# JiehongLin/SAM-6D

Measured on NVIDIA H100. Metric: poses/sec, higher is better.
Workload: dtype bf16

## Files before the change

include/sam6d_b200.h:

```cpp
#ifndef SAM6D_B200_H
#define SAM6D_B200_H

#ifdef __cplusplus
extern "C" {
#endif


int sam6d_fps(const float* xyz, int b, int n, int m, float* temp, int* idx, void* stream);
int sam6d_fps_single_cta(const float* xyz, int b, int n, int m, float* temp, int* idx, void* stream);

int sam6d_gather_points(const float* points, const int* idx, int b, int c, int n, int m, float* out, void* stream);

int sam6d_gather_rows(const float* src, const int* idx, int b, int n, int m, int c, long long src_bstride, float* out,
                      void* stream);
int sam6d_gather_rows_bf16_f32(const void* src, const int* idx, int b, int n, int m, int c, long long src_bstride, float* out,
                               void* stream);

int sam6d_ball_query(const float* new_xyz, const float* xyz, int b, int n, int m, float radius, int nsample, int* idx,
                     int* cnt, void* stream);
int sam6d_ball_query_pair(const float* new_xyz, const float* xyz, int b, int n, int m, float radius_a, int nsample_a,
                          float radius_b, int nsample_b, int* idx_a, int* idx_b, int* cnt_a, int* cnt_b, void* stream);

int sam6d_group_points(const float* points, const int* idx, int b, int c, int n, int np, int ns, float* out, void* stream);

// ... 125 lines not shown
                     float* lse, void* out, int out_is_bf16, long long out_ld, void* stream);
int sam6d_attn_merge_key(const void* Q, long long q_ld, int q_col0, const void* K, long long k_ld, int k_col0, int k_brows,
                         int key_row, const void* Vt, long long vt_ld, int key_col, const float* lse, int B, int H, int Sq,
                         float scale, void* out, long long out_ld, void* stream);
int sam6d_transpose_tokens_bf16(const void* src, long long ld, int col0, int C, int nB, int L, int N1, void* out, void* stream);
int sam6d_linattn_kv(const float* Kf, long long k_ld, long long k_bs, const float* V, long long v_ld, long long v_bs, int B,
                     int H, int J, float* KV, float* KS, void* stream);
int sam6d_linattn_apply(const float* Qf, long long q_rpb, long long q_bs, long long q_ld, const float* KV, const float* KS,
                        int B, int H, float* X, long long x_bs, long long x_ld, void* stream);
int sam6d_linattn_kv_pack(const float* Kf, long long k_ld, long long k_bs, const float* V, long long v_ld, long long v_bs, int B,
                          int J, void* blob, float* KS, void* stream);
int sam6d_linattn_tc(const void* Q, long long q_ld, long long q_bs, const void* blob, const float* KS,
                     const float* softplus_scale, int B, int rpb, void* X, long long x_ld, long long x_bs, void* stream);

int sam6d_coarse_assign(const float* A, int B, int S, float* W, float* w1, void* stream);
int sam6d_coarse_sample(const float* W, int B, int L, const float* rand, int nr, int* idx, void* stream);
int sam6d_coarse_hypotheses(const int* idx, const float* pts1, const float* pts2, int B, int n, int n1, float* Rt,
                            float* resid, void* stream);
int sam6d_topk_smallest(const float* v, int B, int n, int k, int* out, void* stream);
int sam6d_coarse_select(const float* Rt, const int* top, int B, int n1, int n2, const float* pts1, const float* w1, int n,
                        const float* model, int nm, float* scores, float* R, float* t, void* stream);


int sam6d_pe_mlp_max(const float* pts, const int* idx, const int* cnt, int B, int N, int ns, const float* W1,
                     const float* B1, const float* W2, const float* B2, const float* W3, const float* B3, float* out,
                     int out_ld, int out_off, void* stream);
int sam6d_pe_mlp_max_tc(const float* pts, const int* idx, int B, int N, int ns, const float* W1, const float* B1,
                        const void* W2_bf16, const float* B2, const void* W3_bf16, const float* B3, void* out, int out_is_bf16,
                        int out_ld, int out_off, void* stream);
int sam6d_fine_assign(const float* A, int B, int S, int ld, float shift, const float* pts2, float* rsum, float* csum, float* cpart,
                      int* cpi, int* lab1, int* lab2, float* wts, float* pred, void* stream);
int sam6d_fine_pass_tc(const void* Fa, const void* Fb, int B, int S, float alpha, float shift, int mode, const float* row_f,
                       const float* col_f, int ld_f, const float* q4, float* out_inv, int* lab, float* wts, float* pred, void* stream);
int sam6d_fine_masked_points(const int* lab2, const float* pts2, int B, int S, int ld, float* q4, void* stream);
int sam6d_weighted_procrustes(const float* src, const float* ref, const float* wts, int B, int N, float weight_thresh,
                              float eps, float* R, float* t, void* stream);
int sam6d_pose_score(const float* pts1, const int* lab1, int B, int N, const float* R, const float* t, const float* model,
                     int nm, float dis_thres, const float* radius, float* score, float* t_scaled, void* stream);

int sam6d_bilinear_gather(const void* up, int up_is_bf16, const long long* choose, int B, int K, int G, int sub, int C, int H, int W,
                          float* out, void* stream);

int sam6d_attn_relpos(const float* qkv, long long tok_ld, int nW, int Hs, int Ws, int nH, int head_dim, const float* rel_h,
                      const float* rel_w, float scale, void* out, int out_is_bf16, long long out_ld, void* stream);

int sam6d_attn_global_tc(const void* qkv, long long ld, const void* Vt, long long vt_ld, const void* rel_blob, int B, int H, int grid,
                         float scale, void* out, int out_is_bf16, long long out_ld, void* stream);
int sam6d_attn_global_tc_ex(const void* qkv, long long ld, const void* Vt, long long vt_ld, const void* rel_blob, int B, int H, int grid,
                            int head_dim, float scale, void* out, int out_is_bf16, long long out_ld, void* stream);

int sam6d_template_score_agg(const float* Qn, const float* Rn, int P, int O, int T, int C, int aggregation, float* sim_out,
                             float* obj_score, int* obj_tmpl, int* best_obj, float* best_score, int* best_tmpl, void* stream);
int sam6d_template_score(const float* Qn, const float* Rn, int P, int O, int T, int C, float* sim_out, float* obj_score,
                         int* best_obj, float* best_score, int* best_tmpl, void* stream);


int sam6d_render_meshes(const float* verts, const int* faces, const int* mesh_info, int O, int n_verts, int n_faces,
                        const unsigned char* vcol, const float* uv, const unsigned char* tex, const long long* tex_off,
                        const float* base_color, const float* poses, int T, float fx, float fy, float cx, float cy, int H, int W,
                        float znear, float ambient, int* vrec, unsigned long long* vis, int* big, int big_cap, int* counters,
                        unsigned char* rgb, unsigned char* mask, void* xyz, int* tri, float* depth, void* stream);


int sam6d_bop_mssd_mspd(const float* est, const float* gt, const int* pair_obj, const float* K, int P, const float* verts,
                        const int* vert_off, const float* syms, const int* sym_off, int O, int max_sym, float* out, void* stream);
int sam6d_bop_vsd_counts(const float* depth_est, const float* depth_gt, const float* depth_test, const int* pair_img, int P,
// ... 23 lines not shown
```

sam6d_b200/_lib.py:

```python
import ctypes
import os
import re

_HERE = os.path.dirname(os.path.abspath(__file__))
HEADER = os.path.join(os.path.dirname(_HERE), "include", "sam6d_b200.h")
LIB_PATH = os.path.join(_HERE, "libsam6d_b200.so")

_CTYPES = {
    "int": ctypes.c_int,
    "long long": ctypes.c_longlong,
    "float": ctypes.c_float,
    "double": ctypes.c_double,
}


def parse_header(path: str = HEADER):
    text = open(path).read()
    text = re.sub(r"/\*.*?\*/", "", text, flags=re.S)
    protos = {}
    for m in re.finditer(r"(const char\*|int)\s+(sam6d_\w+)\s*\(([^)]*)\)\s*;", text):
        ret, name, args = m.group(1), m.group(2), m.group(3)
        argl = []
        for a in [x.strip() for x in args.split(",")]:
            if a in ("void", ""):
# ... 2 lines not shown
                argl.append((ctypes.c_void_p, a.split("*")[-1].strip()))
            else:
                typ, nm = a.rsplit(" ", 1)
                argl.append((_CTYPES[typ.strip()], nm))
        protos[name] = (ctypes.c_char_p if ret != "int" else ctypes.c_int, argl)
    return protos


class Sam6dError(RuntimeError):
    pass


_lib = None
_protos = None


def lib():
    global _lib, _protos
    if _lib is None:
        if not os.path.exists(LIB_PATH):
            raise Sam6dError(
                f"{LIB_PATH} not found: build it with `python -m sam6d_b200.build` "
                "(or __graft_entry__.build()); sam6d_b200 has no CPU or eager fallback")
        _lib = ctypes.CDLL(LIB_PATH)
        _protos = parse_header()
        for name, (ret, args) in _protos.items():
            fn = getattr(_lib, name)
            fn.restype = ret
            fn.argtypes = [t for t, _ in args]
    return _lib


_launches = 0
_MULTI = {"sam6d_fine_assign": 6, "sam6d_coarse_select": 2, "sam6d_geo_embed_tc": 2, "sam6d_render_meshes": 4, "sam6d_yolo_masks": 2,
          "sam6d_mask_rle_count": 2, "sam6d_template_score_agg": 2, "sam6d_template_score": 2,
          "sam6d_pbr_reference_crops": 2}
_timed = {}


def launch_count() -> int:
    return _launches


def add_launches(n: int):
    global _launches
    _launches += int(n)


def time_kernel(name: str, enable: bool = True):
    if enable:
        _timed[name] = []
    else:
        _timed.pop(name, None)


def timed_events(name: str):
    return _timed.get(name, [])


def call(name: str, *args):
    global _launches
    fn = getattr(lib(), name)
    rec = _timed.get(name)
    if rec is not None:
        import torch
        e0, e1 = torch.cuda.Event(enable_timing=True), torch.cuda.Event(enable_timing=True)
        e0.record()
# ... 16 lines not shown
```

sam6d_b200/csrc/coarse.cu:

```cuda
#include "common.cuh"
#include "svd3.cuh"

namespace {

constexpr int ASSIGN_THREADS = 1024;
__global__ void __launch_bounds__(ASSIGN_THREADS) coarse_assign_kernel(const float* __restrict__ A, int S, float* __restrict__ W,
                                                            float* __restrict__ w1out) {
  extern __shared__ float sm[];
  float* a = sm;
  float* rmax = a + S * S;
  float* rsum = rmax + S;
  float* cmax = rsum + S;
  float* csum = cmax + S;
  int* lab1 = (int*)(csum + S);
  int* lab2 = lab1 + S;
  const int b = blockIdx.x, tid = threadIdx.x, lane = tid & 31, warp = tid >> 5;
  const float* Ab = A + (size_t)b * S * S;
  for (int e = tid; e < S * S; e += ASSIGN_THREADS) a[e] = Ab[e];
  __syncthreads();
  for (int i = warp; i < S; i += ASSIGN_THREADS / 32) {
    float m = -INFINITY;
    for (int j = lane; j < S; j += 32) m = fmaxf(m, a[i * S + j]);
    m = warp_max(m);
    float s = 0.f;
// ... 14 lines not shown
    float v = a[e];
    a[e] = (expf(v - rmax[i]) / rsum[i]) * (expf(v - cmax[j]) / csum[j]);
  }
  __syncthreads();
  for (int i = warp; i < S; i += ASSIGN_THREADS / 32) {
    float bv = -INFINITY; int bi = 0x7fffffff;
    for (int j = lane; j < S; j += 32) argmax_first(bv, bi, a[i * S + j], j);
    warp_argmax_first(bv, bi);
    if (lane == 0) lab1[i] = bi;
  }
  for (int j = tid; j < S; j += ASSIGN_THREADS) {
    float bv = -INFINITY; int bi = 0;
    for (int i = 0; i < S; ++i) { float v = a[i * S + j]; if (v > bv) { bv = v; bi = i; } }
    lab2[j] = bi;
  }
  __syncthreads();
  const int n = S - 1;
  float* Wb = W + (size_t)b * n * n;
  for (int e = tid; e < n * n; e += ASSIGN_THREADS) {
    int i = e / n, j = e - i * n;
    float v = a[(i + 1) * S + (j + 1)];
    v = v * (lab1[i + 1] > 0 ? 1.f : 0.f) * (lab2[j + 1] > 0 ? 1.f : 0.f);
    Wb[e] = v * sqrtf(v);
  }
  for (int i = tid; i < n; i += ASSIGN_THREADS) w1out[(size_t)b * n + i] = lab1[i + 1] > 0 ? 1.f : 0.f;
}

__global__ void __launch_bounds__(1024) coarse_sample_kernel(const float* __restrict__ W, int L, const float* __restrict__ rand,
                                                             int nr, int* __restrict__ idx_out) {
  extern __shared__ float cdf[];
  __shared__ double part[1024];
  const int b = blockIdx.x, tid = threadIdx.x;
  const float* Wb = W + (size_t)b * L;
  const int per = (L + 1023) / 1024;
  const int beg = min(tid * per, L), end = min(beg + per, L);
  double s = 0.0;
  for (int i = beg; i < end; ++i) s += (double)Wb[i];
  part[tid] = s;
  __syncthreads();
  for (int o = 1; o < 1024; o <<= 1) {
    double v = (tid >= o) ? part[tid - o] : 0.0;
    __syncthreads();
    part[tid] += v;
    __syncthreads();
  }
  double run = (tid == 0) ? 0.0 : part[tid - 1];
  for (int i = beg; i < end; ++i) { run += (double)Wb[i]; cdf[i] = (float)run; }
  __syncthreads();
  const float denom = cdf[L - 1] + 1e-8f;
  __syncthreads();
  for (int i = tid; i < L; i += 1024) cdf[i] = cdf[i] / denom;
  __syncthreads();
  for (int r = tid; r < nr; r += 1024) {
    float v = rand[(size_t)b * nr + r];
    int lo = 0, hi = L;
    while (lo < hi) {
      int mid = (lo + hi) >> 1;
      if (cdf[mid] < v) lo = mid + 1; else hi = mid;
    }
    idx_out[(size_t)b * nr + r] = lo;
  }
}

__global__ void __launch_bounds__(128) coarse_hyp_kernel(const int* __restrict__ idx, const float* __restrict__ pts1,
                                                         const float* __restrict__ pts2, int n, int n1, float* __restrict__ Rt,
                                                         float* __restrict__ resid) {
  const int b = blockIdx.y;
  const int hpt = blockIdx.x * blockDim.x + threadIdx.x;
  if (hpt >= n1) return;
  const int* id = idx + ((size_t)b * n1 + hpt) * 3;
  float p1[3][3], p2[3][3];
  int i1s[3], i2s[3];
#pragma unroll
  for (int k = 0; k < 3; ++k) {
    int v = id[k];
    int i1 = min(v / n, n - 1), i2 = min(v % n, n - 1);
    i1s[k] = i1; i2s[k] = i2;
    const float* a = pts1 + ((size_t)b * n + i1) * 3;
    const float* c = pts2 + ((size_t)b * n + i2) * 3;
#pragma unroll
// ... 24 lines not shown
  if (rank0) {
#pragma unroll
    for (int i = 0; i < 3; ++i)
#pragma unroll
      for (int j = 0; j < 3; ++j) Rd[i][j] = (i == j) ? 1.0 : 0.0;
  } else {
    procrustes_rotation(H, Rd, rank1);
  }
  float R[3][3], t[3];
#pragma unroll
  for (int i = 0; i < 3; ++i)
#pragma unroll
    for (int j = 0; j < 3; ++j) R[i][j] = (float)Rd[i][j];
#pragma unroll
  for (int i = 0; i < 3; ++i) t[i] = cr[i] - (R[i][0] * cs[0] + R[i][1] * cs[1] + R[i][2] * cs[2]);
  float rs = 0.f;
#pragma unroll
  for (int k = 0; k < 3; ++k) {
    float x = p1[k][0] - t[0], y = p1[k][1] - t[1], z = p1[k][2] - t[2];
    float ex = x * R[0][0] + y * R[1][0] + z * R[2][0] - p2[k][0];
    float ey = x * R[0][1] + y * R[1][1] + z * R[2][1] - p2[k][1];
    float ez = x * R[0][2] + y * R[1][2] + z * R[2][2] - p2[k][2];
    rs += sqrtf(ex * ex + ey * ey + ez * ez);
  }
  float* o = Rt + ((size_t)b * n1 + hpt) * 12;
#pragma unroll
  for (int i = 0; i < 3; ++i)
#pragma unroll
    for (int j = 0; j < 3; ++j) o[i * 3 + j] = R[i][j];
  o[9] = t[0]; o[10] = t[1]; o[11] = t[2];
  resid[(size_t)b * n1 + hpt] = rs / 3.f;
}

__global__ void __launch_bounds__(1024) topk_smallest_kernel(const float* __restrict__ v, int n, int npow2, int k,
                                                             int* __restrict__ out) {
  extern __shared__ unsigned long long keys[];
  const int b = blockIdx.x, tid = threadIdx.x;
  for (int i = tid; i < npow2; i += 1024) {
    unsigned long long key = ~0ull;
    if (i < n) {
      float f = v[(size_t)b * n + i];
      unsigned u = __float_as_uint(f);
      u = (u & 0x80000000u) ? ~u : (u | 0x80000000u);
      key = ((unsigned long long)u << 32) | (unsigned)i;
    }
    keys[i] = key;
  }
  __syncthreads();
  for (int size = 2; size <= npow2; size <<= 1) {
    for (int stride = size >> 1; stride > 0; stride >>= 1) {
      for (int i = tid; i < npow2 / 2; i += 1024) {
        int lo = 2 * i - (i & (stride - 1));
        int hi = lo + stride;
        bool asc = ((lo & size) == 0);
        unsigned long long a = keys[lo], c = keys[hi];
        if ((a > c) == asc) { keys[lo] = c; keys[hi] = a; }
      }
      __syncthreads();
    }
  }
  for (int i = tid; i < k; i += 1024) out[(size_t)b * k + i] = (int)(keys[i] & 0xffffffffu);
}

constexpr int SEL_PP = 4, SEL_THREADS = 224;
__device__ __forceinline__ float min3f(float a, float b, float c) { return fminf(fminf(a, b), c); }
__global__ void __launch_bounds__(SEL_THREADS) coarse_select_kernel(const float* __restrict__ Rt, const int* __restrict__ top, int n1,
                                                                    int n2, const float* __restrict__ pts1, const float* __restrict__ w1,
                                                                    int n, const float* __restrict__ model, int nm,
                                                                    float* __restrict__ scores) {
  extern __shared__ float4 smq[];
  __shared__ float red[2 * SEL_PP][SEL_THREADS / 32];
  __shared__ float rts[SEL_PP][12];
  const int pose0 = blockIdx.x * SEL_PP, b = blockIdx.y, tid = threadIdx.x;
  for (int i = tid; i < nm; i += SEL_THREADS) {
    const float* q = model + ((size_t)b * nm + i) * 3;
    const float x = q[0], y = q[1], z = q[2];
    smq[i] = make_float4(x, y, z, x * x + y * y + z * z);
  }
  if (tid < SEL_PP * 12) {
    const int pp = tid / 12, e = tid - pp * 12;
    const int pose = min(pose0 + pp, n2 - 1);
    rts[pp][e] = Rt[((size_t)b * n1 + top[(size_t)b * n2 + pose]) * 12 + e];
  }
  __syncthreads();
  float num = 0.f, den[SEL_PP];
#pragma unroll
  for (int pp = 0; pp < SEL_PP; ++pp) den[pp] = 0.f;
  for (int i = tid; i < n; i += SEL_THREADS) {
    const float* p = pts1 + ((size_t)b * n + i) * 3;
    const float px = p[0], py = p[1], pz = p[2];
    float ax[SEL_PP], ay[SEL_PP], az[SEL_PP], x2[SEL_PP], best[SEL_PP];
#pragma unroll
    for (int pp = 0; pp < SEL_PP; ++pp) {
      const float* R = rts[pp];
      const float x = px - R[9], y = py - R[10], z = pz - R[11];
      const float tx = x * R[0] + y * R[3] + z * R[6];
      const float ty = x * R[1] + y * R[4] + z * R[7];
// ... 53 lines not shown
S6_API int sam6d_coarse_assign(const float* A, int B, int S, float* W, float* w1, void* stream) {
  S6_REQUIRE(A && W && w1 && B >= 0 && S >= 2);
  if (B == 0) return 0;
  size_t smem = ((size_t)S * S + 6 * S) * sizeof(float);
  S6_REQUIRE(smem <= 220 * 1024);
  S6_CHECK(cudaFuncSetAttribute(coarse_assign_kernel, cudaFuncAttributeMaxDynamicSharedMemorySize, (int)smem));
  coarse_assign_kernel<<<B, ASSIGN_THREADS, smem, s6_stream(stream)>>>(A, S, W, w1);
  S6_LAUNCH_CHECK();
  return 0;
}

S6_API int sam6d_coarse_sample(const float* W, int B, int L, const float* rand, int nr, int* idx, void* stream) {
  S6_REQUIRE(W && rand && idx && B >= 0 && L > 0 && nr >= 0);
  if (B == 0 || nr == 0) return 0;
  size_t smem = (size_t)L * sizeof(float);
  S6_REQUIRE(smem <= 200 * 1024);
  S6_CHECK(cudaFuncSetAttribute(coarse_sample_kernel, cudaFuncAttributeMaxDynamicSharedMemorySize, (int)smem));
  coarse_sample_kernel<<<B, 1024, smem, s6_stream(stream)>>>(W, L, rand, nr, idx);
  S6_LAUNCH_CHECK();
  return 0;
}

S6_API int sam6d_coarse_hypotheses(const int* idx, const float* pts1, const float* pts2, int B, int n, int n1, float* Rt,
                                   float* resid, void* stream) {
  S6_REQUIRE(idx && pts1 && pts2 && Rt && resid && B >= 0 && n > 0 && n1 >= 0);
  if (B == 0 || n1 == 0) return 0;
  dim3 grid(s6_cdiv(n1, 128), B);
  coarse_hyp_kernel<<<grid, 128, 0, s6_stream(stream)>>>(idx, pts1, pts2, n, n1, Rt, resid);
  S6_LAUNCH_CHECK();
  return 0;
}

S6_API int sam6d_topk_smallest(const float* v, int B, int n, int k, int* out, void* stream) {
  S6_REQUIRE(v && out && B >= 0 && n > 0 && k > 0 && k <= n);
  if (B == 0) return 0;
  int npow2 = 2;
  while (npow2 < n) npow2 <<= 1;
  size_t smem = (size_t)npow2 * sizeof(unsigned long long);
  S6_REQUIRE(smem <= 200 * 1024);
  S6_CHECK(cudaFuncSetAttribute(topk_smallest_kernel, cudaFuncAttributeMaxDynamicSharedMemorySize, (int)smem));
  topk_smallest_kernel<<<B, 1024, smem, s6_stream(stream)>>>(v, n, npow2, k, out);
  S6_LAUNCH_CHECK();
  return 0;
}

S6_API int sam6d_coarse_select(const float* Rt, const int* top, int B, int n1, int n2, const float* pts1, const float* w1, int n,
                               const float* model, int nm, float* scores, float* R, float* t, void* stream) {
  S6_REQUIRE(Rt && top && pts1 && w1 && model && scores && R && t && B >= 0 && n > 0 && nm > 0 && n2 > 0);
  if (B == 0) return 0;
  size_t smem = (size_t)nm * 4 * sizeof(float);
  S6_REQUIRE(smem <= 200 * 1024);
  S6_CHECK(cudaFuncSetAttribute(coarse_select_kernel, cudaFuncAttributeMaxDynamicSharedMemorySize, (int)smem));
  dim3 grid(s6_cdiv(n2, SEL_PP), B);
  coarse_select_kernel<<<grid, SEL_THREADS, smem, s6_stream(stream)>>>(Rt, top, n1, n2, pts1, w1, n, model, nm, scores);
  S6_LAUNCH_CHECK();
  coarse_pick_kernel<<<B, 32, 0, s6_stream(stream)>>>(scores, top, Rt, n1, n2, R, t);
  S6_LAUNCH_CHECK();
  return 0;
}
```

sam6d_b200/csrc/fine_tc.cu:

```cuda
#include "common.cuh"
#include "tc.cuh"

namespace {

constexpr int BM = 128, BN = 256, BK = 64, KB = 4, STAGES = 4;
constexpr int A_KB = BM * BK * 2, B_KB = BN * BK * 2;
constexpr int CONSUMERS = 256, NUM_THREADS = CONSUMERS + 128;
constexpr int SMEM_BYTES = KB * A_KB + STAGES * B_KB + 1024;
constexpr float LOG2E = 1.4426950408889634f;

struct FArgs {
  int B, S, mode, ld_f;
  float a2, s2;
  const float* row_f;
  const float* col_f;
  const float4* q4;
  float* out_inv;
  int* lab;
  float* wts; float* pred;
};

__device__ __forceinline__ float ex2(float x) {
  float y;
  asm("ex2.approx.ftz.f32 %0, %1;" : "=f"(y) : "f"(x));
  return y;
}

template <int MODE>
__global__ void __launch_bounds__(NUM_THREADS, 1) fine_pass_kernel(const __grid_constant__ CUtensorMap tmA, const __grid_constant__ CUtensorMap tmB, FArgs g) {
  extern __shared__ __align__(1024) uint8_t smem_raw[];
  uint8_t* smem = reinterpret_cast<uint8_t*>((reinterpret_cast<uintptr_t>(smem_raw) + 1023) & ~(uintptr_t)1023);
  uint8_t* a_res = smem;
  uint8_t* ring = smem + KB * A_KB;
  __shared__ __align__(8) uint64_t a_full, a_empty, full_bar[STAGES], empty_bar[STAGES];
  __shared__ float sc[2][BN];
  __shared__ __align__(16) float4 sq[2][BN];

  const int tid = threadIdx.x, warp = tid >> 5, lane = tid & 31;
  const int m_tiles = (g.S + BM - 1) / BM, n_tiles = (g.S + BN - 1) / BN;
  const int items = g.B * m_tiles;

  if (tid == 0) {
    tc::mbar_init(&a_full, 1); tc::mbar_init(&a_empty, CONSUMERS / 32);
    for (int s = 0; s < STAGES; ++s) { tc::mbar_init(&full_bar[s], 1); tc::mbar_init(&empty_bar[s], CONSUMERS / 32); }
    tc::mbar_fence_init();
    tc::tma_prefetch_desc(&tmA);
    tc::tma_prefetch_desc(&tmB);
  }
  __syncthreads();

  if (warp >= CONSUMERS / 32) {
    tc::producer_regs();
    if (tid == CONSUMERS) {
      long long gk = 0;
      int it = 0;
      for (int item = blockIdx.x; item < items; item += gridDim.x, ++it) {
        const int b = item / m_tiles, mt = item - b * m_tiles;
        tc::mbar_wait(&a_empty, (uint32_t)((it & 1) ^ 1));
        tc::mbar_arrive_expect_tx(&a_full, KB * A_KB);
        for (int kb = 0; kb < KB; ++kb) tc::tma_load_2d(&tmA, &a_full, a_res + kb * A_KB, kb * BK, b * g.S + mt * BM);
        for (int nt = 0; nt < n_tiles; ++nt)
          for (int kb = 0; kb < KB; ++kb, ++gk) {
            const int s = (int)(gk % STAGES);
            tc::mbar_wait(&empty_bar[s], (uint32_t)(((gk / STAGES) & 1) ^ 1));
            tc::mbar_arrive_expect_tx(&full_bar[s], B_KB);
            tc::tma_load_2d(&tmB, &full_bar[s], ring + s * B_KB, kb * BK, b * g.S + nt * BN);
          }
      }
    }
    return;
  }
  tc::consumer_regs();
  const int wg = warp >> 2, w = warp & 3;
  const uint32_t a_addr = tc::smem_u32(a_res) + wg * (64 * 128);
  long long gk = 0, tcount = 0;
  int it = 0;
  for (int item = blockIdx.x; item < items; item += gridDim.x, ++it) {
    const int b = item / m_tiles, mt = item - b * m_tiles;
    float rf[2] = {0.f, 0.f};
#pragma unroll
    for (int hr = 0; hr < 2; ++hr) {
      const int i = mt * BM + wg * 64 + tc::frag_row(2 * hr, w, lane);
      if (MODE != 0 && i < g.S) rf[hr] = g.row_f[(size_t)b * g.ld_f + i];
    }
    const float* cf = (MODE != 0) ? g.col_f + (size_t)b * g.ld_f : nullptr;
    const float4* q4 = (MODE == 2) ? g.q4 + (size_t)b * g.ld_f : nullptr;
    float sum[2] = {0.f, 0.f}, bv[2] = {-INFINITY, -INFINITY}, ws[2] = {0.f, 0.f}, px[2] = {0.f, 0.f}, py[2] = {0.f, 0.f}, pz[2] = {0.f, 0.f};
    int bi[2] = {0x7fffffff, 0x7fffffff};
    tc::mbar_wait(&a_full, (uint32_t)(it & 1));
    for (int nt = 0; nt < n_tiles; ++nt, ++tcount) {
      const int buf = (int)(tcount & 1);
      if (MODE != 0) {
        const int j = nt * BN + tid;
        sc[buf][tid] = (j < g.S) ? cf[j] : 0.f;
        if (MODE == 2) sq[buf][tid] = (j < g.S) ? q4[j] : make_float4(0.f, 0.f, 0.f, 0.f);
        tc::named_bar(1, CONSUMERS);
      }
      float acc[BN / 2];
      int prev = -1;
      for (int kb = 0; kb < KB; ++kb, ++gk) {
        const int s = (int)(gk % STAGES);
        tc::mbar_wait(&full_bar[s], (uint32_t)((gk / STAGES) & 1));
        const uint32_t b_addr = tc::smem_u32(ring + s * B_KB);
        tc::wg_fence();
#pragma unroll
        for (int k = 0; k < BK / 16; ++k)
          tc::wgmma_bf16<BN>(acc, tc::wg_desc(a_addr + kb * A_KB + k * 32), tc::wg_desc(b_addr + k * 32), (kb | k) ? 1u : 0u);
        tc::wg_commit();
        if (prev >= 0) {
          tc::wg_wait<1>();
          if (lane == 0) tc::mbar_arrive(&empty_bar[prev]);
        }
        prev = s;
      }
      tc::wg_wait<0>();
      if (lane == 0) tc::mbar_arrive(&empty_bar[prev]);
      if (nt == n_tiles - 1 && lane == 0) tc::mbar_arrive(&a_empty);
#pragma unroll
      for (int e = 0; e < BN / 2; ++e) {
        const int hr = (e >> 1) & 1, cl = tc::frag_col(e, lane), j = nt * BN + cl;
        const float ev = (j < g.S) ? ex2(fmaf(acc[e], g.a2, -g.s2)) : 0.f;
        if (MODE == 0) {
          sum[hr] += ev;
        } else {
          const float p = (ev * rf[hr]) * (ev * sc[buf][cl]);
          if (p > bv[hr]) { bv[hr] = p; bi[hr] = j; }
          if (MODE == 2) {
            const float4 q = sq[buf][cl];
            const float pm = p * q.w;
            ws[hr] += pm; px[hr] = fmaf(pm, q.x, px[hr]); py[hr] = fmaf(pm, q.y, py[hr]); pz[hr] = fmaf(pm, q.z, pz[hr]);
          }
        }
      }
    }
#pragma unroll
    for (int hr = 0; hr < 2; ++hr) {
      const int i = mt * BM + wg * 64 + tc::frag_row(2 * hr, w, lane);
      if (MODE == 0) {
        const float t = tc::quad_sum(sum[hr]);
        if ((lane & 3) == 0 && i < g.S) g.out_inv[(size_t)b * g.ld_f + i] = 1.f / t;
      } else {
#pragma unroll
        for (int o = 1; o <= 2; o <<= 1) {
          const float ov = __shfl_xor_sync(0xffffffffu, bv[hr], o);
          const int oi = __shfl_xor_sync(0xffffffffu, bi[hr], o);
          if (ov > bv[hr] || (ov == bv[hr] && oi < bi[hr])) { bv[hr] = ov; bi[hr] = oi; }
        }
        float ww = 0.f, qx = 0.f, qy = 0.f, qz = 0.f;
        if (MODE == 2) { ww = tc::quad_sum(ws[hr]); qx = tc::quad_sum(px[hr]); qy = tc::quad_sum(py[hr]); qz = tc::quad_sum(pz[hr]); }
        if ((lane & 3) == 0 && i < g.S) {
          int lb = bi[hr];
          if (lb == 0x7fffffff) lb = 0;
          g.lab[(size_t)b * g.S + i] = lb;
          if (MODE == 2 && i >= 1) {
            if (lb == 0) { ww = 0.f; qx = 0.f; qy = 0.f; qz = 0.f; }
            const size_t o = (size_t)b * (g.S - 1) + (i - 1);
            const float d = ww + 1e-6f;
            g.wts[o] = ww;
            g.pred[o * 3 + 0] = qx / d; g.pred[o * 3 + 1] = qy / d; g.pred[o * 3 + 2] = qz / d;
          }
        }
      }
    }
  }
}

__global__ void fine_masked_points_kernel(const int* __restrict__ lab2, const float* __restrict__ pts2, int S, int ld, float4* __restrict__ q4) {
  const int b = blockIdx.y, j = blockIdx.x * blockDim.x + threadIdx.x;
  if (j >= ld) return;
  float4 q = make_float4(0.f, 0.f, 0.f, 0.f);
  if (j >= 1 && j < S && lab2[(size_t)b * S + j] > 0) {
    const float* p = pts2 + ((size_t)b * (S - 1) + (j - 1)) * 3;
    q = make_float4(p[0], p[1], p[2], 1.f);
  }
  q4[(size_t)b * ld + j] = q;
}

}

S6_API int sam6d_fine_pass_tc(const void* Fa, const void* Fb, int B, int S, float alpha, float shift, int mode, const float* row_f,
                              const float* col_f, int ld_f, const float* q4, float* out_inv, int* lab, float* wts, float* pred,
                              void* stream) {
  S6_REQUIRE(Fa && Fb && B >= 0 && S >= 2 && mode >= 0 && mode <= 2 && ld_f >= S);
  S6_REQUIRE(((reinterpret_cast<uintptr_t>(Fa) | reinterpret_cast<uintptr_t>(Fb)) & 15) == 0 && (long long)B * S < 2000000000LL);
  if (mode == 0) S6_REQUIRE(out_inv != nullptr);
  if (mode >= 1) S6_REQUIRE(row_f && col_f && lab);
  if (mode == 2) S6_REQUIRE(q4 && wts && pred && (reinterpret_cast<uintptr_t>(q4) & 15) == 0);
  if (B == 0) return 0;
  CUtensorMap tmA, tmB;
  int rc = tc::make_map_2d(&tmA, Fa, (long long)B * S, 256, 256, 64, BM);
  if (rc) return rc;
  rc = tc::make_map_2d(&tmB, Fb, (long long)B * S, 256, 256, 64, BN);
  if (rc) return rc;
  int grid;
  S6_CHECK(s6_persistent_grid(B * s6_cdiv(S, BM), 1, &grid));
  FArgs g{B, S, mode, ld_f, alpha * LOG2E, shift * LOG2E, row_f, col_f, reinterpret_cast<const float4*>(q4), out_inv, lab, wts, pred};
  cudaStream_t st = s6_stream(stream);
#define FINE_LAUNCH(M)                                                                                              \
  do {                                                                                                              \
    S6_CHECK(cudaFuncSetAttribute(fine_pass_kernel<M>, cudaFuncAttributeMaxDynamicSharedMemorySize, SMEM_BYTES));   \
    fine_pass_kernel<M><<<grid, NUM_THREADS, SMEM_BYTES, st>>>(tmA, tmB, g);                                        \
  } while (0)
  if (mode == 0) FINE_LAUNCH(0); else if (mode == 1) FINE_LAUNCH(1); else FINE_LAUNCH(2);
#undef FINE_LAUNCH
  S6_LAUNCH_CHECK();
  return 0;
}

S6_API int sam6d_fine_masked_points(const int* lab2, const float* pts2, int B, int S, int ld, float* q4, void* stream) {
  S6_REQUIRE(lab2 && pts2 && q4 && B >= 0 && S >= 2 && ld >= S && (reinterpret_cast<uintptr_t>(q4) & 15) == 0);
  if (B == 0) return 0;
  dim3 grid(s6_cdiv(ld, 256), B);
  fine_masked_points_kernel<<<grid, 256, 0, s6_stream(stream)>>>(lab2, pts2, S, ld, reinterpret_cast<float4*>(q4));
  S6_LAUNCH_CHECK();
  return 0;
}
```

sam6d_b200/ops.py:

```python
import ctypes
from typing import Optional, Tuple

import torch

from . import _lib

Tensor = torch.Tensor


def _check(t: Tensor, dtype, name: str, ndim: Optional[int] = None):
    if not isinstance(t, torch.Tensor):
        raise RuntimeError(f"{name} must be a torch.Tensor")
    if not t.is_cuda:
        raise RuntimeError(f"{name} must be a CUDA tensor (CPU not supported)")
    if t.dtype != dtype:
        raise RuntimeError(f"{name} must be {dtype}, got {t.dtype}")
    if not t.is_contiguous():
        raise RuntimeError(f"{name} must be contiguous")
    if ndim is not None and t.dim() != ndim:
        raise RuntimeError(f"{name} must have {ndim} dims, got {t.dim()}")


def _p(t: Optional[Tensor]):
    return ctypes.c_void_p(0 if t is None else t.data_ptr())
# ... 643 lines not shown
        ld = (S + 3) // 4 * 4
        store = torch.empty(B, S, ld, dtype=torch.float32, device=A.device)
        store[:, :, :S] = A
        A = store[:, :, :S]
    ld = A.stride(1)
    dev = A.device
    tiles = (S + 31) // 32
    if tiles < 4:
        raise RuntimeError("fine_assign: S >= 97 required")
    rsum = torch.empty(B, ld, dtype=torch.float32, device=dev)
    csum = torch.empty(B, ld, dtype=torch.float32, device=dev)
    cpart = torch.empty(B, tiles, ld, dtype=torch.float32, device=dev)
    cpi = torch.empty(B, tiles, ld, dtype=torch.int32, device=dev)
    lab1 = torch.zeros(B, S, dtype=torch.int32, device=dev)
    lab2 = torch.zeros(B, S, dtype=torch.int32, device=dev)
    wts = torch.empty(B, S - 1, dtype=torch.float32, device=dev)
    pred = torch.empty(B, S - 1, 3, dtype=torch.float32, device=dev)
    _lib.call("sam6d_fine_assign", _p(A), B, S, int(ld), _f(shift), _p(pts2), _p(rsum), _p(csum), _p(cpart), _p(cpi), _p(lab1),
              _p(lab2), _p(wts), _p(pred), _s())
    return lab1, lab2, wts, pred


def fine_assign_tc(f1n: Tensor, f2n: Tensor, pts2: Tensor, alpha: float):
    _check(f1n, torch.bfloat16, "f1n", 3)
    _check(f2n, torch.bfloat16, "f2n", 3)
    _check(pts2, torch.float32, "pts2", 3)
    B, S, C = f1n.shape
    if C != 256 or f2n.shape != f1n.shape or pts2.shape[1] != S - 1:
        raise RuntimeError("fine_assign_tc: (B,S,256) tokens and (B,S-1,3) points expected")
    dev = f1n.device
    ld = (S + 3) // 4 * 4
    rinv = torch.empty(B, ld, dtype=torch.float32, device=dev)
    cinv = torch.empty(B, ld, dtype=torch.float32, device=dev)
    q4 = torch.empty(B, ld, 4, dtype=torch.float32, device=dev)
    lab1 = torch.zeros(B, S, dtype=torch.int32, device=dev)
    lab2 = torch.zeros(B, S, dtype=torch.int32, device=dev)
    wts = torch.empty(B, S - 1, dtype=torch.float32, device=dev)
    pred = torch.empty(B, S - 1, 3, dtype=torch.float32, device=dev)
    a, sh = _f(alpha), _f(alpha)
    _lib.call("sam6d_fine_pass_tc", _p(f1n), _p(f2n), B, S, a, sh, 0, None, None, ld, None, _p(rinv), None, None, None, _s())
    _lib.call("sam6d_fine_pass_tc", _p(f2n), _p(f1n), B, S, a, sh, 0, None, None, ld, None, _p(cinv), None, None, None, _s())
    _lib.call("sam6d_fine_pass_tc", _p(f2n), _p(f1n), B, S, a, sh, 1, _p(cinv), _p(rinv), ld, None, None, _p(lab2), None, None, _s())
    _lib.call("sam6d_fine_masked_points", _p(lab2), _p(pts2), B, S, ld, _p(q4), _s())
    _lib.call("sam6d_fine_pass_tc", _p(f1n), _p(f2n), B, S, a, sh, 2, _p(rinv), _p(cinv), ld, _p(q4), None, _p(lab1), _p(wts), _p(pred),
              _s())
    return lab1, lab2, wts, pred


def weighted_procrustes(src: Tensor, ref: Tensor, wts: Tensor, weight_thresh: float = 0.0, eps: float = 1e-5):
    _check(src, torch.float32, "src", 3)
    _check(ref, torch.float32, "ref", 3)
    _check(wts, torch.float32, "weights", 2)
    B, N, _ = src.shape
    R = torch.empty(B, 3, 3, dtype=torch.float32, device=src.device)
    t = torch.empty(B, 3, dtype=torch.float32, device=src.device)
    _lib.call("sam6d_weighted_procrustes", _p(src), _p(ref), _p(wts), B, N, _f(weight_thresh), _f(eps), _p(R), _p(t), _s())
    return R, t


def pose_score(pts1: Tensor, lab1: Tensor, R: Tensor, t: Tensor, model: Tensor, radius: Tensor, dis_thres: float = 0.15):
    _check(pts1, torch.float32, "pts1", 3)
    _check(lab1, torch.int32, "lab1", 2)
    B, N, _ = pts1.shape
    score = torch.empty(B, dtype=torch.float32, device=pts1.device)
    ts = torch.empty(B, 3, dtype=torch.float32, device=pts1.device)
    _lib.call("sam6d_pose_score", _p(pts1), _p(lab1), B, N, _p(R), _p(t), _p(model), model.shape[1], _f(dis_thres),
              _p(radius), _p(score), _p(ts), _s())
    return score, ts


def attn_relpos(qkv: Tensor, nW: int, Hs: int, Ws: int, nH: int, rel_h: Tensor, rel_w: Tensor, scale: float,
                out_dtype=torch.float32) -> Tensor:
    _check(qkv, torch.float32, "qkv", 2)
    _check(rel_h, torch.float32, "rel_pos_h", 2)
# ... 59 lines not shown
```

Measured before the change: 2648.

## Fuse fine row/col softmax sums, radix-select topk, stage coarse CDF in smem

Adds a MODE 3 fine pass that computes row sums and per-tile column partial sums from one GEMM sweep, plus a small reduction kernel, replacing two separate full score-matrix passes. Replaces the bitonic-sort top-k with an 8-bit radix select over 48-bit keys followed by rank placement of the k survivors. The coarse sampling CDF now loads weights into shared memory once instead of reading global memory twice, and SEL_PP changes from 4 to 5. In exchange the fused pass does extra shuffles and shared-memory reductions, top-k now requires n <= 65536, and the final rank step is O(k^2) per batch.

```diff
diff --git a/include/sam6d_b200.h b/include/sam6d_b200.h
--- a/include/sam6d_b200.h
+++ b/include/sam6d_b200.h
@@ -181,6 +181,8 @@
                       int* cpi, int* lab1, int* lab2, float* wts, float* pred, void* stream);
 int sam6d_fine_pass_tc(const void* Fa, const void* Fb, int B, int S, float alpha, float shift, int mode, const float* row_f,
                        const float* col_f, int ld_f, const float* q4, float* out_inv, int* lab, float* wts, float* pred, void* stream);
+int sam6d_fine_sums_tc(const void* Fa, const void* Fb, int B, int S, float alpha, float shift, int ld_f, float* cpart,
+                       float* rinv, float* cinv, void* stream);
 int sam6d_fine_masked_points(const int* lab2, const float* pts2, int B, int S, int ld, float* q4, void* stream);
 int sam6d_weighted_procrustes(const float* src, const float* ref, const float* wts, int B, int N, float weight_thresh,
                               float eps, float* R, float* t, void* stream);
diff --git a/sam6d_b200/_lib.py b/sam6d_b200/_lib.py
--- a/sam6d_b200/_lib.py
+++ b/sam6d_b200/_lib.py
@@ -58,7 +58,7 @@
 
 
 _launches = 0
-_MULTI = {"sam6d_fine_assign": 6, "sam6d_coarse_select": 2, "sam6d_geo_embed_tc": 2, "sam6d_render_meshes": 4, "sam6d_yolo_masks": 2,
+_MULTI = {"sam6d_fine_assign": 6, "sam6d_fine_sums_tc": 2, "sam6d_coarse_select": 2, "sam6d_geo_embed_tc": 2, "sam6d_render_meshes": 4, "sam6d_yolo_masks": 2,
           "sam6d_mask_rle_count": 2, "sam6d_template_score_agg": 2, "sam6d_template_score": 2,
           "sam6d_pbr_reference_crops": 2}
 _timed = {}
diff --git a/sam6d_b200/csrc/coarse.cu b/sam6d_b200/csrc/coarse.cu
--- a/sam6d_b200/csrc/coarse.cu
+++ b/sam6d_b200/csrc/coarse.cu
@@ -70,10 +70,12 @@
   __shared__ double part[1024];
   const int b = blockIdx.x, tid = threadIdx.x;
   const float* Wb = W + (size_t)b * L;
+  for (int i = tid; i < L; i += 1024) cdf[i] = Wb[i];
+  __syncthreads();
   const int per = (L + 1023) / 1024;
   const int beg = min(tid * per, L), end = min(beg + per, L);
   double s = 0.0;
-  for (int i = beg; i < end; ++i) s += (double)Wb[i];
+  for (int i = beg; i < end; ++i) s += (double)cdf[i];
   part[tid] = s;
   __syncthreads();
   for (int o = 1; o < 1024; o <<= 1) {
@@ -83,7 +85,7 @@
     __syncthreads();
   }
   double run = (tid == 0) ? 0.0 : part[tid - 1];
-  for (int i = beg; i < end; ++i) { run += (double)Wb[i]; cdf[i] = (float)run; }
+  for (int i = beg; i < end; ++i) { run += (double)cdf[i]; cdf[i] = (float)run; }
   __syncthreads();
   const float denom = cdf[L - 1] + 1e-8f;
   __syncthreads();
@@ -174,37 +176,69 @@
   resid[(size_t)b * n1 + hpt] = rs / 3.f;
 }
 
-__global__ void __launch_bounds__(1024) topk_smallest_kernel(const float* __restrict__ v, int n, int npow2, int k,
-                                                             int* __restrict__ out) {
+constexpr int TOPK_THREADS = 1024;
+__global__ void __launch_bounds__(TOPK_THREADS) topk_smallest_kernel(const float* __restrict__ v, int n, int k, int* __restrict__ out) {
   extern __shared__ unsigned long long keys[];
-  const int b = blockIdx.x, tid = threadIdx.x;
-  for (int i = tid; i < npow2; i += 1024) {
-    unsigned long long key = ~0ull;
-    if (i < n) {
-      float f = v[(size_t)b * n + i];
-      unsigned u = __float_as_uint(f);
-      u = (u & 0x80000000u) ? ~u : (u | 0x80000000u);
-      key = ((unsigned long long)u << 32) | (unsigned)i;
-    }
-    keys[i] = key;
-  }
-  __syncthreads();
-  for (int size = 2; size <= npow2; size <<= 1) {
-    for (int stride = size >> 1; stride > 0; stride >>= 1) {
-      for (int i = tid; i < npow2 / 2; i += 1024) {
-        int lo = 2 * i - (i & (stride - 1));
-        int hi = lo + stride;
-        bool asc = ((lo & size) == 0);
-        unsigned long long a = keys[lo], c = keys[hi];
-        if ((a > c) == asc) { keys[lo] = c; keys[hi] = a; }
+  unsigned long long* sel = keys + n;
+  __shared__ unsigned hist[256];
+  __shared__ unsigned long long s_prefix;
+  __shared__ unsigned s_rank, s_count;
+  const int b = blockIdx.x, tid = threadIdx.x, lane = tid & 31;
+  for (int i = tid; i < n; i += TOPK_THREADS) {
+    unsigned u = __float_as_uint(v[(size_t)b * n + i]);
+    u = (u & 0x80000000u) ? ~u : (u | 0x80000000u);
+    keys[i] = ((unsigned long long)u << 16) | (unsigned)i;
+  }
+  if (tid == 0) s_count = 0;
+  unsigned long long prefix = 0;
+  unsigned rank = (unsigned)k;
+  for (int shift = 40; shift >= 0; shift -= 8) {
+    if (tid < 256) hist[tid] = 0;
+    __syncthreads();
+    const unsigned long long hmask = ~0ull << (shift + 8);
+    for (int i = tid; i < n; i += TOPK_THREADS) {
+      const unsigned long long key = keys[i];
+      if ((key & hmask) == prefix) atomicAdd(&hist[(key >> shift) & 255], 1u);
+    }
+    __syncthreads();
+    if (tid < 32) {
+      unsigned c[8], tot = 0;
+#pragma unroll
+      for (int q = 0; q < 8; ++q) { c[q] = hist[lane * 8 + q]; tot += c[q]; }
+      unsigned incl = tot;
+#pragma unroll
+      for (int o = 1; o < 32; o <<= 1) {
+        const unsigned y = __shfl_up_sync(0xffffffffu, incl, o);
+        if (lane >= o) incl += y;
       }
-      __syncthreads();
-    }
-  }
-  for (int i = tid; i < k; i += 1024) out[(size_t)b * k + i] = (int)(keys[i] & 0xffffffffu);
-}
-
-constexpr int SEL_PP = 4, SEL_THREADS = 224;
+      unsigned before = incl - tot;
+#pragma unroll
+      for (int q = 0; q < 8; ++q) {
+        if (before < rank && rank <= before + c[q]) {
+          s_prefix = prefix | ((unsigned long long)(lane * 8 + q) << shift);
+          s_rank = rank - before;
+        }
+        before += c[q];
+      }
+    }
+    __syncthreads();
+    prefix = s_prefix;
+    rank = s_rank;
+  }
+  for (int i = tid; i < n; i += TOPK_THREADS) {
+    const unsigned long long key = keys[i];
+    if (key <= prefix) sel[atomicAdd(&s_count, 1u)] = key;
+  }
+  __syncthreads();
+  for (int t = tid; t < k; t += TOPK_THREADS) {
+    const unsigned long long key = sel[t];
+    int r = 0;
+    for (int u = 0; u < k; ++u) r += sel[u] < key;
+    out[(size_t)b * k + r] = (int)(key & 0xffffu);
+  }
+}
+
+constexpr int SEL_PP = 5, SEL_THREADS = 224;
 __device__ __forceinline__ float min3f(float a, float b, float c) { return fminf(fminf(a, b), c); }
 __global__ void __launch_bounds__(SEL_THREADS) coarse_select_kernel(const float* __restrict__ Rt, const int* __restrict__ top, int n1,
                                                                     int n2, const float* __restrict__ pts1, const float* __restrict__ w1,
@@ -324,14 +358,12 @@
 }
 
 S6_API int sam6d_topk_smallest(const float* v, int B, int n, int k, int* out, void* stream) {
-  S6_REQUIRE(v && out && B >= 0 && n > 0 && k > 0 && k <= n);
+  S6_REQUIRE(v && out && B >= 0 && n > 0 && k > 0 && k <= n && n <= 65536);
   if (B == 0) return 0;
-  int npow2 = 2;
-  while (npow2 < n) npow2 <<= 1;
-  size_t smem = (size_t)npow2 * sizeof(unsigned long long);
+  size_t smem = (size_t)(n + k) * sizeof(unsigned long long);
   S6_REQUIRE(smem <= 200 * 1024);
   S6_CHECK(cudaFuncSetAttribute(topk_smallest_kernel, cudaFuncAttributeMaxDynamicSharedMemorySize, (int)smem));
-  topk_smallest_kernel<<<B, 1024, smem, s6_stream(stream)>>>(v, n, npow2, k, out);
+  topk_smallest_kernel<<<B, TOPK_THREADS, smem, s6_stream(stream)>>>(v, n, k, out);
   S6_LAUNCH_CHECK();
   return 0;
 }
diff --git a/sam6d_b200/csrc/fine_tc.cu b/sam6d_b200/csrc/fine_tc.cu
--- a/sam6d_b200/csrc/fine_tc.cu
+++ b/sam6d_b200/csrc/fine_tc.cu
@@ -16,6 +16,7 @@
   const float* col_f;
   const float4* q4;
   float* out_inv;
+  float* cpart;
   int* lab;
   float* wts; float* pred;
 };
@@ -35,6 +36,7 @@
   __shared__ __align__(8) uint64_t a_full, a_empty, full_bar[STAGES], empty_bar[STAGES];
   __shared__ float sc[2][BN];
   __shared__ __align__(16) float4 sq[2][BN];
+  __shared__ __align__(16) float cred[MODE == 3 ? 2 : 1][MODE == 3 ? CONSUMERS / 32 : 1][BN];
 
   const int tid = threadIdx.x, warp = tid >> 5, lane = tid & 31;
   const int m_tiles = (g.S + BM - 1) / BM, n_tiles = (g.S + BN - 1) / BN;
@@ -72,25 +74,28 @@
   }
   tc::consumer_regs();
   const int wg = warp >> 2, w = warp & 3;
+  constexpr bool ROWSUM = (MODE == 0 || MODE == 3);
   const uint32_t a_addr = tc::smem_u32(a_res) + wg * (64 * 128);
   long long gk = 0, tcount = 0;
   int it = 0;
   for (int item = blockIdx.x; item < items; item += gridDim.x, ++it) {
     const int b = item / m_tiles, mt = item - b * m_tiles;
     float rf[2] = {0.f, 0.f};
+    bool rv[2];
 #pragma unroll
     for (int hr = 0; hr < 2; ++hr) {
       const int i = mt * BM + wg * 64 + tc::frag_row(2 * hr, w, lane);
-      if (MODE != 0 && i < g.S) rf[hr] = g.row_f[(size_t)b * g.ld_f + i];
-    }
-    const float* cf = (MODE != 0) ? g.col_f + (size_t)b * g.ld_f : nullptr;
+      rv[hr] = i < g.S;
+      if (!ROWSUM && i < g.S) rf[hr] = g.row_f[(size_t)b * g.ld_f + i];
+    }
+    const float* cf = (!ROWSUM) ? g.col_f + (size_t)b * g.ld_f : nullptr;
     const float4* q4 = (MODE == 2) ? g.q4 + (size_t)b * g.ld_f : nullptr;
     float sum[2] = {0.f, 0.f}, bv[2] = {-INFINITY, -INFINITY}, ws[2] = {0.f, 0.f}, px[2] = {0.f, 0.f}, py[2] = {0.f, 0.f}, pz[2] = {0.f, 0.f};
     int bi[2] = {0x7fffffff, 0x7fffffff};
     tc::mbar_wait(&a_full, (uint32_t)(it & 1));
     for (int nt = 0; nt < n_tiles; ++nt, ++tcount) {
       const int buf = (int)(tcount & 1);
-      if (MODE != 0) {
+      if (!ROWSUM) {
         const int j = nt * BN + tid;
         sc[buf][tid] = (j < g.S) ? cf[j] : 0.f;
         if (MODE == 2) sq[buf][tid] = (j < g.S) ? q4[j] : make_float4(0.f, 0.f, 0.f, 0.f);
@@ -117,26 +122,61 @@
       if (lane == 0) tc::mbar_arrive(&empty_bar[prev]);
       if (nt == n_tiles - 1 && lane == 0) tc::mbar_arrive(&a_empty);
 #pragma unroll
-      for (int e = 0; e < BN / 2; ++e) {
-        const int hr = (e >> 1) & 1, cl = tc::frag_col(e, lane), j = nt * BN + cl;
-        const float ev = (j < g.S) ? ex2(fmaf(acc[e], g.a2, -g.s2)) : 0.f;
-        if (MODE == 0) {
-          sum[hr] += ev;
-        } else {
-          const float p = (ev * rf[hr]) * (ev * sc[buf][cl]);
-          if (p > bv[hr]) { bv[hr] = p; bi[hr] = j; }
-          if (MODE == 2) {
-            const float4 q = sq[buf][cl];
-            const float pm = p * q.w;
-            ws[hr] += pm; px[hr] = fmaf(pm, q.x, px[hr]); py[hr] = fmaf(pm, q.y, py[hr]); pz[hr] = fmaf(pm, q.z, pz[hr]);
-          }
+      for (int kk = 0; kk < 4; ++kk) {
+        float cv[16];
+#pragma unroll
+        for (int e = kk * 32; e < kk * 32 + 32; ++e) {
+          const int hr = (e >> 1) & 1, cl = tc::frag_col(e, lane), j = nt * BN + cl;
+          const float ev = (j < g.S) ? ex2(fmaf(acc[e], g.a2, -g.s2)) : 0.f;
+          if (ROWSUM) {
+            sum[hr] += ev;
+            if (MODE == 3) {
+              const int sl = ((e >> 2) & 7) * 2 + (e & 1);
+              const float cvv = rv[hr] ? ev : 0.f;
+              if (hr == 0) cv[sl] = cvv; else cv[sl] += cvv;
+            }
+          } else {
+            const float p = (ev * rf[hr]) * (ev * sc[buf][cl]);
+            if (p > bv[hr]) { bv[hr] = p; bi[hr] = j; }
+            if (MODE == 2) {
+              const float4 q = sq[buf][cl];
+              const float pm = p * q.w;
+              ws[hr] += pm; px[hr] = fmaf(pm, q.x, px[hr]); py[hr] = fmaf(pm, q.y, py[hr]); pz[hr] = fmaf(pm, q.z, pz[hr]);
+            }
+          }
+        }
+        if (MODE == 3) {
+#pragma unroll
+          for (int step = 4; step >= 1; step >>= 1) {
+            const bool up = (lane & (4 * step)) != 0;
+#pragma unroll
+            for (int o = 0; o < step; ++o)
+#pragma unroll
+              for (int c = 0; c < 2; ++c) {
+                const float lo = cv[o * 2 + c], hi = cv[(o + step) * 2 + c];
+                const float recv = __shfl_xor_sync(0xffffffffu, up ? lo : hi, 4 * step);
+                cv[o * 2 + c] = (up ? hi : lo) + recv;
+              }
+          }
+          *reinterpret_cast<float2*>(&cred[buf][warp][(kk * 8 + (lane >> 2)) * 8 + 2 * (lane & 3)]) = make_float2(cv[0], cv[1]);
+        }
+      }
+      if (MODE == 3) {
+        tc::named_bar(2 + wg, 128);
+        const int t = tid - 128 * wg;
+        float* cp = g.cpart + ((size_t)(b * m_tiles + mt) * 2 + wg) * g.ld_f;
+#pragma unroll
+        for (int h = 0; h < 2; ++h) {
+          const int c = t + 128 * h, j = nt * BN + c;
+          const float s = ((cred[buf][4 * wg][c] + cred[buf][4 * wg + 1][c]) + cred[buf][4 * wg + 2][c]) + cred[buf][4 * wg + 3][c];
+          if (j < g.S) cp[j] = s;
         }
       }
     }
 #pragma unroll
     for (int hr = 0; hr < 2; ++hr) {
       const int i = mt * BM + wg * 64 + tc::frag_row(2 * hr, w, lane);
-      if (MODE == 0) {
+      if (ROWSUM) {
         const float t = tc::quad_sum(sum[hr]);
         if ((lane & 3) == 0 && i < g.S) g.out_inv[(size_t)b * g.ld_f + i] = 1.f / t;
       } else {
@@ -176,17 +216,20 @@
   q4[(size_t)b * ld + j] = q;
 }
 
-}
-
-S6_API int sam6d_fine_pass_tc(const void* Fa, const void* Fb, int B, int S, float alpha, float shift, int mode, const float* row_f,
-                              const float* col_f, int ld_f, const float* q4, float* out_inv, int* lab, float* wts, float* pred,
-                              void* stream) {
-  S6_REQUIRE(Fa && Fb && B >= 0 && S >= 2 && mode >= 0 && mode <= 2 && ld_f >= S);
+__global__ void fine_col_inv_kernel(const float* __restrict__ cpart, int parts, int S, int ld, float* __restrict__ inv) {
+  const int b = blockIdx.y, j = blockIdx.x * blockDim.x + threadIdx.x;
+  if (j >= S) return;
+  const float* p = cpart + (size_t)b * parts * ld + j;
+  float s = 0.f;
+  for (int k = 0; k < parts; ++k) s += p[(size_t)k * ld];
+  inv[(size_t)b * ld + j] = 1.f / s;
+}
+
+}
+
+static int fine_launch(const void* Fa, const void* Fb, int B, int S, float alpha, float shift, int ld_f, const FArgs& g0,
+                       cudaStream_t st) {
   S6_REQUIRE(((reinterpret_cast<uintptr_t>(Fa) | reinterpret_cast<uintptr_t>(Fb)) & 15) == 0 && (long long)B * S < 2000000000LL);
-  if (mode == 0) S6_REQUIRE(out_inv != nullptr);
-  if (mode >= 1) S6_REQUIRE(row_f && col_f && lab);
-  if (mode == 2) S6_REQUIRE(q4 && wts && pred && (reinterpret_cast<uintptr_t>(q4) & 15) == 0);
-  if (B == 0) return 0;
   CUtensorMap tmA, tmB;
   int rc = tc::make_map_2d(&tmA, Fa, (long long)B * S, 256, 256, 64, BM);
   if (rc) return rc;
@@ -194,15 +237,48 @@
   if (rc) return rc;
   int grid;
   S6_CHECK(s6_persistent_grid(B * s6_cdiv(S, BM), 1, &grid));
-  FArgs g{B, S, mode, ld_f, alpha * LOG2E, shift * LOG2E, row_f, col_f, reinterpret_cast<const float4*>(q4), out_inv, lab, wts, pred};
-  cudaStream_t st = s6_stream(stream);
+  FArgs g = g0;
+  g.B = B; g.S = S; g.ld_f = ld_f; g.a2 = alpha * LOG2E; g.s2 = shift * LOG2E;
 #define FINE_LAUNCH(M)                                                                                              \
   do {                                                                                                              \
     S6_CHECK(cudaFuncSetAttribute(fine_pass_kernel<M>, cudaFuncAttributeMaxDynamicSharedMemorySize, SMEM_BYTES));   \
     fine_pass_kernel<M><<<grid, NUM_THREADS, SMEM_BYTES, st>>>(tmA, tmB, g);                                        \
   } while (0)
-  if (mode == 0) FINE_LAUNCH(0); else if (mode == 1) FINE_LAUNCH(1); else FINE_LAUNCH(2);
+  switch (g.mode) {
+    case 0: FINE_LAUNCH(0); break;
+    case 1: FINE_LAUNCH(1); break;
+    case 2: FINE_LAUNCH(2); break;
+    default: FINE_LAUNCH(3); break;
+  }
 #undef FINE_LAUNCH
+  S6_LAUNCH_CHECK();
+  return 0;
+}
+
+S6_API int sam6d_fine_pass_tc(const void* Fa, const void* Fb, int B, int S, float alpha, float shift, int mode, const float* row_f,
+                              const float* col_f, int ld_f, const float* q4, float* out_inv, int* lab, float* wts, float* pred,
+                              void* stream) {
+  S6_REQUIRE(Fa && Fb && B >= 0 && S >= 2 && mode >= 0 && mode <= 2 && ld_f >= S);
+  if (mode == 0) S6_REQUIRE(out_inv != nullptr);
+  if (mode >= 1) S6_REQUIRE(row_f && col_f && lab);
+  if (mode == 2) S6_REQUIRE(q4 && wts && pred && (reinterpret_cast<uintptr_t>(q4) & 15) == 0);
+  if (B == 0) return 0;
+  FArgs g{};
+  g.mode = mode; g.row_f = row_f; g.col_f = col_f; g.q4 = reinterpret_cast<const float4*>(q4);
+  g.out_inv = out_inv; g.lab = lab; g.wts = wts; g.pred = pred;
+  return fine_launch(Fa, Fb, B, S, alpha, shift, ld_f, g, s6_stream(stream));
+}
+
+S6_API int sam6d_fine_sums_tc(const void* Fa, const void* Fb, int B, int S, float alpha, float shift, int ld_f, float* cpart,
+                              float* rinv, float* cinv, void* stream) {
+  S6_REQUIRE(Fa && Fb && cpart && rinv && cinv && B >= 0 && S >= 2 && ld_f >= S);
+  if (B == 0) return 0;
+  FArgs g{};
+  g.mode = 3; g.out_inv = rinv; g.cpart = cpart;
+  cudaStream_t st = s6_stream(stream);
+  const int rc = fine_launch(Fa, Fb, B, S, alpha, shift, ld_f, g, st);
+  if (rc) return rc;
+  fine_col_inv_kernel<<<dim3(s6_cdiv(S, 256), B), 256, 0, st>>>(cpart, 2 * s6_cdiv(S, BM), S, ld_f, cinv);
   S6_LAUNCH_CHECK();
   return 0;
 }
diff --git a/sam6d_b200/ops.py b/sam6d_b200/ops.py
--- a/sam6d_b200/ops.py
+++ b/sam6d_b200/ops.py
@@ -699,14 +699,14 @@
     ld = (S + 3) // 4 * 4
     rinv = torch.empty(B, ld, dtype=torch.float32, device=dev)
     cinv = torch.empty(B, ld, dtype=torch.float32, device=dev)
+    cpart = torch.empty(B, 2 * ((S + 127) // 128), ld, dtype=torch.float32, device=dev)
     q4 = torch.empty(B, ld, 4, dtype=torch.float32, device=dev)
     lab1 = torch.zeros(B, S, dtype=torch.int32, device=dev)
     lab2 = torch.zeros(B, S, dtype=torch.int32, device=dev)
     wts = torch.empty(B, S - 1, dtype=torch.float32, device=dev)
     pred = torch.empty(B, S - 1, 3, dtype=torch.float32, device=dev)
     a, sh = _f(alpha), _f(alpha)
-    _lib.call("sam6d_fine_pass_tc", _p(f1n), _p(f2n), B, S, a, sh, 0, None, None, ld, None, _p(rinv), None, None, None, _s())
-    _lib.call("sam6d_fine_pass_tc", _p(f2n), _p(f1n), B, S, a, sh, 0, None, None, ld, None, _p(cinv), None, None, None, _s())
+    _lib.call("sam6d_fine_sums_tc", _p(f1n), _p(f2n), B, S, a, sh, ld, _p(cpart), _p(rinv), _p(cinv), _s())
     _lib.call("sam6d_fine_pass_tc", _p(f2n), _p(f1n), B, S, a, sh, 1, _p(cinv), _p(rinv), ld, None, None, _p(lab2), None, None, _s())
     _lib.call("sam6d_fine_masked_points", _p(lab2), _p(pts2), B, S, ld, _p(q4), _s())
     _lib.call("sam6d_fine_pass_tc", _p(f1n), _p(f2n), B, S, a, sh, 2, _p(rinv), _p(cinv), ld, _p(q4), None, _p(lab1), _p(wts), _p(pred),
```

Result: faster. 2725 (median of 6 runs) (+2.9%).
